# mako443/Text2Pos-CVPR2022

Hardware: AMD Instinct MI355X
Metric: cells+queries encoded/sec and top-k retrieval QPS, 256-pt cells, 12k-cell DB (higher is better)
Workload: dtype f16x3 (fp32 operands split hi+lo into fp16, 3 f16 MFMAs, fp32 accumulate; fp32-class error) for the encoders / f64 MFMA for the ranking

## Files before the change

### include/t2p.h

```cpp
#ifndef T2P_H
#define T2P_H
#include <stddef.h>
#include <stdint.h>

#ifdef __cplusplus
extern "C" {
#endif

#define T2P_ABI_VERSION 31
#define T2P_DEFAULT_CHUNK_OBJECTS 65000
#define T2P_MAX_CHUNK_OBJECTS 65535
#define T2P_TUNING_MASK 0x5
#define T2P_E_ARG (-1)
#define T2P_E_WORKSPACE (-2)
#define T2P_E_UNSUPPORTED (-3)

typedef void* t2p_stream_t;

int t2p_abi_version(void);
const char* t2p_last_error(void);

typedef struct t2p_cell_weights {
    const float* sa_w1[3];
    const float* sa_b1[3];
    const float* sa_w2[3];
    const float* sa_b2[3];
    const float* ga_w1;
    const float* ga_b1;
    const float* ga_w2;
    const float* ga_b2;
    const float* lin1_w;
    const float* lin1_b;
    const float* lin2_w;
    const float* lin2_b;
    const float* pn_w;
    const float* pn_b;
    const float* col_w1;
    const float* col_b1;
    const float* col_w2;
    const float* col_b2;
    const float* pos_w1;
    const float* pos_b1;
    const float* pos_w2;
    const float* pos_b2;
    const float* merge_w;
// ... 224 lines not shown
```

### profiles/tail_rows_census.py

```python
#!/usr/bin/env python
import argparse
import os
import sys

import numpy as np

sys.path.insert(0, os.path.join(os.path.dirname(os.path.abspath(__file__)), ".."))

RADII = (0.2, 0.3, 0.4)
MAX_NBR = 32


def level(pos: np.ndarray, r: float):
    n_d = pos.shape[0]
    n_c = (n_d + 1) // 2
    r2 = np.float32(r) * np.float32(r)
    mind = np.full(n_d, np.inf, dtype=np.float32)
    fps = np.zeros(n_c, dtype=np.int64)
    cnt = np.zeros(n_c, dtype=np.int64)
    cur = 0
    for c in range(n_c):
        fps[c] = cur
        d = pos - pos[cur]
        d2 = (d[:, 0] * d[:, 0] + d[:, 1] * d[:, 1]) + d[:, 2] * d[:, 2]
        cnt[c] = min(int((d2 < r2).sum()), MAX_NBR)
        mind = np.minimum(mind, d2)
        cur = int(np.argmax(mind))
    return fps, cnt


def dedup_hits(pos: np.ndarray, rgb: np.ndarray, fps: np.ndarray, r: float) -> int:
    key = np.concatenate([pos, rgb], axis=1).view(np.uint32)
    _, first = np.unique(key, axis=0, return_index=True)
    orig = np.zeros(pos.shape[0], dtype=bool)
    orig[first] = True
    r2 = np.float32(r) * np.float32(r)
    kept = 0
    for c in fps:
        d = pos - pos[c]
        d2 = (d[:, 0] * d[:, 0] + d[:, 1] * d[:, 1]) + d[:, 2] * d[:, 2]
        hits = np.flatnonzero(d2 < r2)[:MAX_NBR]
        kept += int(orig[hits].sum())
    return kept


def main():
    ap = argparse.ArgumentParser(description=__doc__.split("\n")[0])
    ap.add_argument("--seed", type=int, default=20220002, help="bench.py's object stream")
    ap.add_argument("--objects", type=int, default=3000)
    args = ap.parse_args()
    from importlib import import_module
    S = import_module("text2pos-cvpr2022_amd.synthetic")
    xyz, rgb, _, _ = S.make_objects(args.seed, 0, args.objects)
    n = xyz.shape[0]
    rows = np.zeros(3)
    rows_dedup = 0.0
    with_tail = np.zeros(3)
    tail_cent = np.zeros(3)
    tail_rows = np.zeros(3)
    executed = np.zeros(3)
    cents = np.zeros(3)
    for o in range(n):
        pos = xyz[o].astype(np.float32)
        for l in range(3):
            fps, cnt = level(pos, RADII[l])
            n_c = fps.shape[0]
            tail = (fps == 0) & (np.arange(n_c) > 0)
            all_rows = cnt.sum() + n_c
            t_rows = cnt[tail].sum()
            rows[l] += all_rows
            cents[l] += n_c
            with_tail[l] += tail.any()
            tail_cent[l] += tail.sum()
            tail_rows[l] += t_rows
            executed[l] += all_rows - t_rows + (cnt[0] if tail.any() else 0)
            if l == 0:
                rows_dedup += dedup_hits(pos, rgb[o].astype(np.float32), fps, RADII[0]) + n_c
            pos = pos[fps]
    print(f"{n} objects of seed {args.seed}")
    print("level | rows/object | objects with a tail | tail centroids | tail rows (non-self) | rows/object, tail shared")
    for l in range(3):
        extra = f" ({rows_dedup / n:.0f} after point dedup)" if l == 0 else ""
        print(f"SA{l + 1}   | {rows[l] / n:8.0f}{extra} | {100 * with_tail[l] / n:5.1f} % | {100 * tail_cent[l] / cents[l]:5.1f} % | "
              f"{100 * tail_rows[l] / rows[l]:5.1f} % | {executed[l] / n:8.0f} ({100 * (executed[l] / rows[l] - 1):+.1f} %)")


if __name__ == "__main__":
    main()
```

### text2pos-cvpr2022_amd/csrc/api.hip

```cpp
#include <stdarg.h>
#include <stdlib.h>
#include <string.h>

#include <mutex>
#include <set>
#include <utility>

#include "../../include/t2p.h"
#include "t2p_common.h"

namespace t2p {

static thread_local char g_err[512] = "";

void set_error(const char* fmt, ...) {
    va_list ap;
    va_start(ap, fmt);
    vsnprintf(g_err, sizeof(g_err), fmt, ap);
    va_end(ap);
}

int num_cus() {
    static int cached = 0;
    if (cached == 0) {
// ... 243 lines not shown
        GroupTables gt = ws.gt;
        const bool want_nbr = tr != nullptr && (tr->nbr[0] || tr->nbr[1] || tr->nbr[2] || tr->cnt[0] || tr->cnt[1] || tr->cnt[2]);
        if (!want_nbr)
            for (int l = 0; l < 3; l++) gt.nbr[l] = gt.cnt[l] = nullptr;
        for (int l = 0; l < 3; l++) {
            const int cf = l == 0 ? 3 : Geo::C[l - 1];
            gt.B[l] = lds_btab[l] ? nullptr : ws.B[l];
            gt.wp[l] = W.sa_w1[l] + (size_t)cf * Geo::H[l];
            gt.H[l] = Geo::H[l];
            gt.tail[l] = ws.F[l];
            gt.ld_tail[l] = Geo::LD[l];
            gt.tail_col0[l] = Geo::C[l];
        }
        gt.tail_rows[2] = g.gp;
        gt.A1 = sa1_points ? nullptr : ws.A[0];
        gt.w1 = W.sa_w1[0];
        gt.b1 = W.sa_b1[0];
        gt.rgb = rgb;
        gt.H1 = Geo::H[0];
        gt.guard = guard;

        SaParams bp[3] = {};
        for (int l = 0; l < 3; l++) {
            bp[l].n_rows = gt.n_rows[l];
            bp[l].n_obj = n;
            bp[l].prefix_ws = ws.prefix[l];
            bp[l].bounds_ws = ws.bounds[l];
            bp[l].W_x3 = cfg.precision == 1 ? W.sa_w2_x3[l] : nullptr;
            bp[l].wp = lds_btab[l] ? W.sa_w1[l] : nullptr;
            bp[l].n_dense = g.nd[l];
            bp[l].n_cent = g.nc[l];
        }
        bp[0].w1 = sa1_points ? W.sa_w1[0] : nullptr;
        for (int l = 0; l < 3; l++) gt.share_tail[l] = sa_shares_tail_rows(l, Geo::H[l], Geo::C[l], bp[l], cfg.n_pts, cfg.tuning) ? 1 : 0;

        T2P_TRY(launch_sample_group(xyz, n, cfg.n_pts, cfg.radius, gt, st));
        if (!(cfg.tuning & 1) && cfg.n_pts == 256)
            T2P_TRY(launch_dedup_rows(xyz, rgb, n, cfg.n_pts, gt.rows[0], gt.n_rows[0], g.nc[0], st));
        T2P_TRY(launch_sa_balance_levels(bp, Geo::H, Geo::C, st));
    }

    for (int l = 0; l < 3; l++) {
        const int H = Geo::H[l], C = Geo::C[l];
        const int cf = l == 0 ? 3 : Geo::C[l - 1];
        const float* pos_src = l == 0 ? xyz : ws.F[l - 1];
        const int ld_pos = l == 0 ? 3 : Geo::LD[l - 1];
        const int pos_col0 = l == 0 ? 0 : Geo::C[l - 1];
        if (l != 0) {
            WsParams p{};
            p.A = ws.F[l - 1];
            p.lda = Geo::LD[l - 1];
            p.k_live = Geo::C[l - 1] + 4;
            p.W = W.sa_w1[l];
            p.W_x3 = cfg.precision == 1 ? W.sa_w1_x3[l] : nullptr;
            p.ldw = H;
            p.bias = W.sa_b1[l];
            p.out = ws.A[l];
            p.ldo = H;
            p.relu = 0;
            p.M = n * g.nd[l];
            p.amax_out = gslot(l == 1 ? G_A2 : G_A3);
            T2P_TRY(launch_ws(WS_DENSE_STORE, Geo::LD[l - 1] - (cfg.precision == 1 ? 16 : 0), H, p, st));
        }
        SaParams p{};
        p.A = ws.A[l];
        p.Bc = ws.B[l];
        p.wp = lds_btab[l] ? W.sa_w1[l] + (size_t)cf * Geo::H[l] : nullptr;
// ... 651 lines not shown
    for (int l = 0; l < 3; l++) {
        gt.fps_idx[l] = fps_idx[l];
        gt.nbr[l] = nbr[l];
        gt.cnt[l] = cnt[l];
        gt.rows[l] = nullptr;
        gt.n_rows[l] = nullptr;
        gt.n_dense[l] = g.nd[l];
        gt.n_cent[l] = g.nc[l];
    }
    return launch_sample_group(xyz, n_obj, n_pts, radius_host, gt, (hipStream_t)stream);
}

int t2p_group_rows(const float* xyz, int64_t n_obj, int32_t n_pts, const float* radius_host, int32_t self_loops,
                   uint8_t* const* fps_idx, uint16_t* const* rows, uint16_t* const* n_rows, t2p_stream_t stream) {
    T2P_CHECK_ARG(xyz && radius_host && fps_idx && rows && n_rows, "group_rows: NULL argument");
    Geo g(n_pts);
    GroupTables gt{};
    gt.self_loops = self_loops ? 1 : 0;
    for (int l = 0; l < 3; l++) {
        T2P_CHECK_ARG(fps_idx[l] && rows[l] && n_rows[l], "group_rows: NULL table of level %d", l);
        gt.fps_idx[l] = fps_idx[l];
        gt.rows[l] = rows[l];
        gt.n_rows[l] = n_rows[l];
        gt.n_dense[l] = g.nd[l];
        gt.n_cent[l] = g.nc[l];
    }
    return launch_sample_group(xyz, n_obj, n_pts, radius_host, gt, (hipStream_t)stream);
}

int t2p_group_rows_shared(const float* xyz, int64_t n_obj, int32_t n_pts, const float* radius_host, int32_t self_loops,
                          int32_t share_mask, uint8_t* const* fps_idx, uint16_t* const* rows, uint16_t* const* n_rows,
                          t2p_stream_t stream) {
    T2P_CHECK_ARG(xyz && radius_host && fps_idx && rows && n_rows, "group_rows_shared: NULL argument");
    T2P_CHECK_ARG((share_mask & ~2) == 0, "group_rows_shared: share_mask=%#x (bit 1: SA level 2; no other level has a shared form)", share_mask);
    T2P_CHECK_ARG(share_mask == 0 || n_pts == 256, "group_rows_shared: shared lists exist for 256 points per object (n_pts = %d)", n_pts);
    Geo g(n_pts);
    GroupTables gt{};
    gt.self_loops = self_loops ? 1 : 0;
    for (int l = 0; l < 3; l++) {
        T2P_CHECK_ARG(fps_idx[l] && rows[l] && n_rows[l], "group_rows_shared: NULL table of level %d", l);
        gt.fps_idx[l] = fps_idx[l];
        gt.rows[l] = rows[l];
        gt.n_rows[l] = n_rows[l];
        gt.n_dense[l] = g.nd[l];
        gt.n_cent[l] = g.nc[l];
        gt.share_tail[l] = (share_mask >> l) & 1;
    }
    return launch_sample_group(xyz, n_obj, n_pts, radius_host, gt, (hipStream_t)stream);
}

int t2p_edge_counts(const uint16_t* rows, const uint16_t* n_rows, const int32_t* first_obj, int64_t n_obj, int32_t n_dense,
                    int32_t n_cent, int32_t self_loops, int32_t* counts, t2p_stream_t stream) {
    T2P_CHECK_ARG(n_obj >= 0 && (n_obj == 0 || (rows && n_rows && first_obj && counts)), "edge_counts: NULL argument");
    return launch_edge_counts(rows, n_rows, first_obj, n_obj, n_dense, n_cent, self_loops, counts, (hipStream_t)stream);
}

int t2p_edge_expand(const uint16_t* rows, const uint16_t* n_rows, const int32_t* first_obj, const int32_t* cent_ptr, int64_t n_obj,
                    int32_t n_dense, int32_t n_cent, int32_t self_loops, int32_t* src, int32_t* dst, t2p_stream_t stream) {
    T2P_CHECK_ARG(n_obj >= 0 && (n_obj == 0 || (rows && n_rows && first_obj && cent_ptr)), "edge_expand: NULL argument");
    return launch_edge_expand(rows, n_rows, first_obj, cent_ptr, n_obj, n_dense, n_cent, self_loops, src, dst, (hipStream_t)stream);
}

int t2p_pack_objects(const float* raw_xyz, const float* raw_rgb, const int32_t* obj_ptr, const int32_t* sample_idx,
                     const float* rot_cos_sin, int64_t n_obj, int32_t n_pts, float* xyz, float* rgb, float* center, float* mean_rgb,
                     t2p_stream_t stream) {
    T2P_CHECK_ARG(raw_xyz && raw_rgb && obj_ptr && sample_idx && xyz && rgb && center && mean_rgb, "pack_objects: NULL argument");
    T2P_CHECK_ARG(n_obj >= 0 && n_pts >= 1, "pack_objects: bad sizes");
// ... 53 lines not shown
```

### text2pos-cvpr2022_amd/csrc/sa_points.hip

```cpp
#ifndef T2P_PABL
#define T2P_PABL 0
#endif
#include "t2p_common.h"

namespace t2p {
namespace {

typedef uint32_t u32x4 __attribute__((ext_vector_type(4)));
typedef uint32_t u32x2 __attribute__((ext_vector_type(2)));
typedef float f32x2 __attribute__((ext_vector_type(2)));

#define MFMA16(a, b, c) __builtin_amdgcn_mfma_f32_32x32x16_f16(a, b, c, 0, 0, 0)
#define MFMA8(a, b, c) __builtin_amdgcn_mfma_f32_32x32x8f16(a, b, c, 0, 0, 0)

template <int NW>
struct PtsCfg {
    static constexpr int K = 32, N = 64, NC = 128, ND = 256, GS = 16;
    static constexpr int NT = 64 * NW;
    static constexpr int S16 = K / 16, NTW = N / 32;
    static constexpr int HS = GS / 2, NH = NC / HS;
    static constexpr int MAXR = NC * 33;
    static constexpr int LPR = 64 / HS;
    static constexpr int ACC_BYTES = GS * N * 4;
    static constexpr int PTS_BYTES = ND * 24;
    static constexpr int SELF_BYTES = GS * 24;
    static constexpr int CEN_BYTES = GS * 32;
    static constexpr int RING_BYTES = 4 * 64 * 2;
    static constexpr int WAVE_BYTES = ACC_BYTES + PTS_BYTES + SELF_BYTES + CEN_BYTES + 16 + 64 + RING_BYTES;
    static_assert(WAVE_BYTES % 16 == 0, "16-byte accesses");
    static constexpr size_t lds_bytes() { return (size_t)NW * WAVE_BYTES + 16 + N * 4; }
};

__device__ __forceinline__ float relu1(float v) {
    const int b = __float_as_int(v);
    return __int_as_float(b > 0 ? b : 0);
}
__device__ __forceinline__ void split2(float v0, float v1, uint32_t& hi, uint32_t& lo) {
    const fp16x2 hh = cvt_pk_f16(v0, v1);
    const fp16x2 ll = cvt_pk_f16(sub_half<0>(v0, hh), sub_half<1>(v1, hh));
    hi = __builtin_bit_cast(uint32_t, hh);
    lo = __builtin_bit_cast(uint32_t, ll);
}

template <int NW, int PARTS>
__global__ __launch_bounds__(64 * NW, (NW + 3) / 4) void k_sa_points(SaParams p) {
    using C = PtsCfg<NW>;
    static_assert(PARTS == 1 || (C::NH % PARTS == 0 && C::NH / PARTS >= 3), "a part is a whole number (>= 3: two open + one fetched ahead) of halves");
    constexpr int K = C::K, N = C::N, NC = C::NC;
    extern __shared__ __attribute__((aligned(16))) char lds[];
    const int tid = threadIdx.x, lane = tid & 63;
    const int wave = __builtin_amdgcn_readfirstlane(tid >> 6);
    const int h = lane >> 5, rr = lane & 31;
    const uint32_t acc_off = (uint32_t)(wave * C::WAVE_BYTES);
    const uint32_t pts_off = acc_off + C::ACC_BYTES;
    const uint32_t self_off = pts_off + C::PTS_BYTES;
    const uint32_t cen_off = self_off + C::SELF_BYTES;
    const uint32_t one_off = cen_off + C::CEN_BYTES;
    const uint32_t dst_off = one_off + 16;
    const uint32_t ring_off = dst_off + 64;
    if (lane == 0) *(f32x4*)(lds + one_off) = f32x4{1.f, 0.f, 0.f, 0.f};

    half8 w_hi[C::NTW][C::S16], w_lo[C::NTW][C::S16];
    {
        const uint4* wp = (const uint4*)p.W_x3;
        constexpr int PLANE_U4 = (N / 32) * C::S16 * 64;
#pragma unroll
        for (int nt = 0; nt < C::NTW; nt++)
#pragma unroll
            for (int s = 0; s < C::S16; s++) {
                uint4 pc[2][2];
#pragma unroll
                for (int hp = 0; hp < 2; hp++) {
                    const int kb = 16 * s + 8 * hp;
                    const int half_ = kb / (K / 2), step_ = (kb % (K / 2)) / 8;
                    const int idx = (((nt * C::S16 + step_) * 2 + half_) * 32) + rr;
                    pc[0][hp] = wp[idx];
                    pc[1][hp] = wp[PLANE_U4 + idx];
                }
                const u32x4 vh = h ? u32x4{pc[0][0].z, pc[0][0].w, pc[0][1].z, pc[0][1].w} : u32x4{pc[0][0].x, pc[0][0].y, pc[0][1].x, pc[0][1].y};
                const u32x4 vl = h ? u32x4{pc[1][0].z, pc[1][0].w, pc[1][1].z, pc[1][1].w} : u32x4{pc[1][0].x, pc[1][0].y, pc[1][1].x, pc[1][1].y};
                w_hi[nt][s] = __builtin_bit_cast(half8, vh);
                w_lo[nt][s] = __builtin_bit_cast(half8, vl);
            }
    }
    half4 w1_hi, w1_lo;
    {
        float wv[4];
#pragma unroll
        for (int e = 0; e < 4; e++) {
            const int k = 4 * h + e;
            wv[e] = k < 6 ? p.w1[k * K + rr] : (k == 6 ? p.b1[rr] : 0.f);
        }
// ... 26 lines not shown
        const int g = g_begin + (PARTS > 1 ? gi / PARTS : gi);
        if (g >= g_end) break;
        constexpr int HP = C::NH / PARTS;
        const int hs = PARTS > 1 ? (gi % PARTS) * HP : 0;
        const int hend = hs + HP;
        int n = __builtin_amdgcn_readfirstlane((int)p.n_rows[g]);
        const uint16_t* list = p.rows + (int64_t)g * C::MAXR;
        if constexpr (PARTS > 1) {
            auto lower = [&](int target) -> int {
                if (target <= 0 || n <= 0) return 0;
                if (target >= NC) return n;
                const int step = (n + 63) >> 6;
                const int i0 = lane * step;
                const uint32_t c0 = i0 < n ? (((uint32_t)list[i0] >> 8) & 127u) : 255u;
                const unsigned long long ge = __ballot(c0 >= (uint32_t)target);
                const int fl = ge ? (int)__builtin_ctzll(ge) : 64;
                if (fl == 0) return 0;
                int hi = fl * step;
                hi = hi < n ? hi : n;
                const int base = (fl - 1) * step + 1;
                for (int b = base; b < hi; b += 64) {
                    const int i = b + lane;
                    const uint32_t c = i < hi ? (((uint32_t)list[i] >> 8) & 127u) : 255u;
                    const unsigned long long m = __ballot(c >= (uint32_t)target);
                    if (m) return b + (int)__builtin_ctzll(m);
                }
                return hi;
            };
            const int r_lo = __builtin_amdgcn_readfirstlane(lower(hs * C::HS));
            const int r_hi = __builtin_amdgcn_readfirstlane(lower(hend * C::HS));
            list += r_lo;
            n = r_hi - r_lo;
        }
        const int first = __builtin_amdgcn_readfirstlane(p.first[g]);
        const uint32_t sb0 = (uint32_t)(first * C::ND + (g - first) * NC);

        const int nwin = (n + 63) >> 6;
        auto load_win = [&](int w) -> uint32_t {
            int i = w * 64 + lane;
            i = i < n ? i : n - 1;
            i = i > 0 ? i : 0;
            return (uint32_t)list[i];
        };
        auto ring_write = [&](int w, uint32_t v) { *(uint16_t*)(lds + ring_off + (((w & 3) * 64 + lane) * 2)) = (uint16_t)v; };
        auto ring_read = [&](int r) -> uint32_t {
            return (uint32_t) * (const uint16_t*)(lds + ring_off + (((r + rr) & 255) * 2));
        };
        const uint32_t win0 = load_win(0), win1 = load_win(1);
        uint32_t pend = load_win(2);
        int w_loaded = 2;

        typedef float f32x3 __attribute__((ext_vector_type(3)));
        struct Side { f32x3 q, sp, sc; };
        auto fetch_side = [&](int hh) -> Side {
            const int c = hh * C::HS + (lane & (C::HS - 1));
            const float* pc = p.out + ((int64_t)g * NC + c) * (int64_t)p.ldo + N;
            const int64_t ai = (int64_t)sb0 + c;
            return Side{*(const f32x3*)pc, *(const f32x3*)(p.pos_src + ai * 3), *(const f32x3*)(p.feat_src + ai * 3)};
        };
        const Side side0 = fetch_side(hs), side1 = fetch_side(hs + 1);

        {
            const f32x4* px4 = (const f32x4*)(p.pos_src + (int64_t)g * C::ND * 3) + lane * 3;
            const f32x4* pc4 = (const f32x4*)(p.feat_src + (int64_t)g * C::ND * 3) + lane * 3;
            const f32x4 a0 = px4[0], a1 = px4[1], a2 = px4[2];
            const f32x4 c0_ = pc4[0], c1_ = pc4[1], c2_ = pc4[2];
            f32x4* rec = (f32x4*)(lds + pts_off + lane * 96);
            rec[0] = f32x4{c0_[0], c0_[1], c0_[2], a0[0]};
            rec[1] = f32x4{a0[1], a0[2], c0_[3], c1_[0]};
            rec[2] = f32x4{c1_[1], a0[3], a1[0], a1[1]};
            rec[3] = f32x4{c1_[2], c1_[3], c2_[0], a1[2]};
            rec[4] = f32x4{a1[3], a2[0], c2_[1], c2_[2]};
            rec[5] = f32x4{c2_[3], a2[1], a2[2], a2[3]};
        }
        ring_write(0, win0);
        ring_write(1, win1);

        auto flush_out = [&]() {
            if (has_pout) {
#pragma unroll
                for (int q4 = 0; q4 < NPL / 4; q4++) *(f32x4*)(pptr + q4 * 4) = pout[q4];
                has_pout = false;
            }
        };
        auto drain = [&](int hh, bool live) {
            flush_out();
            pptr = p.out + ((int64_t)g * NC + hh * C::HS + cr) * (int64_t)p.ldo + cs * NPL;
            const uint32_t a0 = acc_off + (uint32_t)((((hh & 1) * C::HS + cr) * N + cs * NPL) * 4);
            int top = gtop;
#pragma unroll
            for (int q4 = 0; q4 < NPL / 4; q4++) {
                f32x4 v = f32x4{0.f, 0.f, 0.f, 0.f};
                if (live) {
                    const f32x4 raw = *(const f32x4*)(lds + a0 + q4 * 16);
                    const f32x4 bq = *(const f32x4*)(lds + bias_off + q4 * 16);
#pragma unroll
                    for (int e = 0; e < 4; e++) {
                        const float r = fmaxf(raw[e] + bq[e], 0.f);
                        const int bits = __float_as_int(r);
                        top = bits > top ? bits : top;
                        v[e] = r * p.out_scale;
                    }
                }
                pout[q4] = v;
            }
            has_pout = true;
            gtop = top;
        };
        auto open_half = [&](int hh, const Side& sd) {
            const uint32_t s0 = (uint32_t)((hh & 1) * C::HS);
            if (lane < C::HS) {
                uint2* sp = (uint2*)(lds + self_off + (s0 + lane) * 24);
                sp[0] = uint2{__float_as_uint(sd.sc[0]), __float_as_uint(sd.sc[1])};
                sp[1] = uint2{__float_as_uint(sd.sc[2]), __float_as_uint(sd.sp[0])};
                sp[2] = uint2{__float_as_uint(sd.sp[1]), __float_as_uint(sd.sp[2])};
                f32x4* cp = (f32x4*)(lds + cen_off + (s0 + lane) * 32);
                cp[0] = f32x4{0.f, 0.f, 0.f, sd.q[0]};
                cp[1] = f32x4{sd.q[1], sd.q[2], 0.f, 0.f};
            }
            typedef int i32x4 __attribute__((ext_vector_type(4)));
            const uint32_t a0 = acc_off + (uint32_t)(((s0 + cr) * N + cs * NPL) * 4);
#pragma unroll
            for (int q4 = 0; q4 < NPL / 4; q4++)
                *(i32x4*)(lds + a0 + q4 * 16) = i32x4{(int)0xFF800000, (int)0xFF800000, (int)0xFF800000, (int)0xFF800000};
        };

        open_half(hs, side0);
        open_half(hs + 1, side1);
        Side side_n = fetch_side(hs + 2);
        int hf = hs + 2;
        int hd = hs, ho = hs + 2;
        int r0 = 0;
        uint32_t e_cur = n > 0 ? ring_read(0) : 0u;
        while (r0 < n) {
            const uint32_t key = r0 + rr < n ? ((e_cur >> 8) & 127u) : 255u;
            const int h0 = __builtin_amdgcn_readfirstlane((int)key) >> 3;
            const uint32_t over = (uint32_t)__ballot(key >= (uint32_t)((h0 + 2) * C::HS));
            const int c = over ? (int)__builtin_ctz(over) : 32;
            const uint32_t e_nxt = ring_read(r0 + c);
            if (hd < h0 || ho < h0 + 2) {
                if (hd < h0) asm volatile("s_waitcnt lgkmcnt(0)" ::: "memory");
                while (hd < h0) {
                    drain(hd, hd < ho);
                    hd++;
                }
                if (ho < hd) ho = hd;
                const int want = h0 + 2 < hend ? h0 + 2 : hend;
                while (ho < want) {
                    if (hf != ho) side_n = fetch_side(ho);
                    open_half(ho, side_n);
                    ho++;
                    if (ho < hend) {
                        side_n = fetch_side(ho);
                        hf = ho;
                    }
                }
            }
            if (w_loaded * 64 < r0 + 96 && w_loaded < nwin) {
                ring_write(w_loaded, pend);
                w_loaded++;
                flush_out();
                if (w_loaded < nwin) pend = load_win(w_loaded);
            }
            const uint32_t m = rr < c ? e_cur : (uint32_t)__builtin_amdgcn_readlane((int)e_cur, c - 1);
            const uint32_t src = m & 0xFFu, d = m >> 8;
            const uint32_t dl = d & 15u;
            const uint32_t rec = (d & 0x80u) ? self_off + dl * 24u : pts_off + src * 24u;
            const uint32_t pa0 = rec + (uint32_t)(h * 16), pa1 = h ? one_off : rec + 8u;
            f32x4 pv, cv;
            if constexpr (T2P_PABL & 8) {
                pv = f32x4{(float)pa0, 1.f, 2.f, (float)pa1};
                cv = f32x4{(float)dl, 1.f, 2.f, 3.f};
            } else {
                const f32x2 p0 = *(const f32x2*)(lds + pa0), p1 = *(const f32x2*)(lds + pa1);
                pv = f32x4{p0[0], p0[1], p1[0], p1[1]};
                cv = *(const f32x4*)(lds + cen_off + dl * 32u + (uint32_t)(h * 16));
            }
            *(uint16_t*)(lds + dst_off + rr * 2) = (uint16_t)(dl * (uint32_t)(N * 4));
            uint32_t xh[2], xl[2];
            split2(pv[0] - cv[0], pv[1] - cv[1], xh[0], xl[0]);
            split2(pv[2] - cv[2], pv[3] - cv[3], xh[1], xl[1]);
            const half4 x_hi = __builtin_bit_cast(half4, u32x2{xh[0], xh[1]});
            const half4 x_lo = __builtin_bit_cast(half4, u32x2{xl[0], xl[1]});
            f32x16 hid;
            if constexpr (T2P_PABL & 4) {
#pragma unroll
                for (int e = 0; e < 16; e++) hid[e] = (float)x_hi[e & 3] + (float)x_lo[e & 3];
            } else {
// ... 36 lines not shown
                    const uint32_t pair = (e & 2) ? four[e >> 2].y : four[e >> 2].x;
                    ad[e] = acc_off + (uint32_t)(rr * 4) + ((e & 1) ? (pair >> 16) : (pair & 0xFFFFu));
                }
                static_assert(C::NTW == 2, "the hazard fence below names both result blocks");
                asm volatile("s_nop 15" : "+v"(acc[0]), "+v"(acc[1])::"memory");
#pragma unroll
                for (int nt = 0; nt < C::NTW; nt++)
#pragma unroll
                    for (int e = 0; e < 16; e++)
                        if constexpr (!(T2P_PABL & 1))
                            asm volatile("ds_max_f32 %0, %1 offset:%2" ::"v"(ad[e]), "v"(acc[nt][e]), "n"(nt * 128) : "memory");
                        else
                            asm volatile("; %0 %1" ::"v"(ad[e]), "v"(acc[nt][e]));
            }
            r0 += c;
            e_cur = e_nxt;
        }
        asm volatile("s_waitcnt lgkmcnt(0)" ::: "memory");
        for (; hd < hend; hd++) drain(hd, hd < ho);
        flush_out();
    }
    uint32_t gbits = 0;
    guard_track_bits(gbits, gtop);
    if (p.amax_out != nullptr && lane == 0 && gbits != 0u)
        atomicMax(p.amax_out, __float_as_uint(__uint_as_float(gbits) * p.out_scale));
}

#ifndef T2P_PTS_WAVES
#define T2P_PTS_WAVES 12
#endif
constexpr int kPtsWaves = T2P_PTS_WAVES;
constexpr int kPtsParts = 4;

}

bool sa_points_selected(int H, int Cout, const SaParams& p) {
    return H == 32 && Cout == 64 && p.W_x3 != nullptr && p.wp != nullptr && p.w1 != nullptr;
}

int sa_points_launch_shape(int64_t n_obj, int* tile_rows, int* n_wg) {
    int n = num_cus();
    if (n > 1024) n = 1024;
    if (n > n_obj) n = (int)n_obj;
    *tile_rows = 32;
    *n_wg = n;
    return 0;
}

int launch_sa_points(int H, int Cout, const SaParams& p, hipStream_t st) {
    if (!(H == 32 && Cout == 64 && p.n_cent == 128 && p.n_dense == 256 && p.wp && p.W_x3 && p.w1 && p.b1 && p.feat_src && p.pos_src &&
          p.ld_pos == 3 && p.pos_col0 == 0)) {
        set_error("sa_points: built for SA level 1 (6 -> 32 -> 64, 128 centroids of 256 points [xyz] + [rgb], f16x3)");
        return T2P_E_UNSUPPORTED;
    }
    using C = PtsCfg<kPtsWaves>;
    auto kern = k_sa_points<kPtsWaves, 1>, kern_parts = k_sa_points<kPtsWaves, kPtsParts>;
    T2P_TRY(reserve_lds((const void*)kern, C::lds_bytes(), "sa_points"));
    T2P_TRY(reserve_lds((const void*)kern_parts, C::lds_bytes(), "sa_points"));
    if (p.n_obj <= 0) return 0;
    T2P_CHECK_ARG(p.n_obj < (1 << 22), "sa_points: chunk too large");
    T2P_CHECK_ARG((((uintptr_t)p.pos_src | (uintptr_t)p.feat_src | (uintptr_t)p.out | (uintptr_t)p.W_x3) & 15) == 0 && p.ldo % 4 == 0,
                  "sa_points: points, output rows and weights must be 16-byte aligned");
    int tr, n_wg;
    sa_points_launch_shape(p.n_obj, &tr, &n_wg);
    if (!p.balanced) T2P_TRY(launch_sa_balance(p, tr, n_wg, st));
    ProfScope ps_("ws_edge_sa_k32_n64", st);
    const bool parts = p.n_obj * 2 <= (int64_t)n_wg * kPtsWaves;
    T2P_REPEAT(ps_) hipLaunchKernelGGL(parts ? kern_parts : kern, dim3(n_wg), dim3(C::NT), C::lds_bytes(), st, p);
    T2P_CHECK_LAUNCH("sa_points");
    return 0;
}

}
```

### text2pos-cvpr2022_amd/csrc/sample_group.hip

```cpp
#include "t2p_common.h"

namespace t2p {

#pragma clang fp contract(off)

namespace {

#ifndef T2P_FPS_PK
#define T2P_FPS_PK 1
#endif

constexpr int kMaxPts = 256;
constexpr int kMaxNbr = 32;

__device__ __forceinline__ float dist2(float ax, float ay, float az, float bx, float by, float bz) {
#pragma clang fp contract(off)
    float dx = ax - bx, dy = ay - by, dz = az - bz;
    float xx = dx * dx, yy = dy * dy, zz = dz * dz;
    float s = xx + yy;
    return s + zz;
}

template <int CTRL>
__device__ __forceinline__ int dpp_i(int v) {
// ... 78 lines not shown
            lower = __builtin_amdgcn_mbcnt_hi((uint32_t)(m >> 32), __builtin_amdgcn_mbcnt_lo((uint32_t)m, lower));
            count += __popcll(m);
        }
        int pos = lower;
#pragma unroll
        for (int j = 0; j < PPL; j++) {
            if (hit[j] && pos < kMaxNbr) {
                const int i = lane * PPL + j;
                if (nbr_lds) nbr_lds[c * kMaxNbr + pos] = (uint8_t)i;
                if (rows_out) rows_out[base + pos] = (uint16_t)((c << 8) | i);
            }
            pos += hit[j] ? 1 : 0;
        }
        const int kept = count < kMaxNbr ? count : kMaxNbr;
        if (lane == 0) {
            if (nbr_lds) cnt_lds[c] = (uint8_t)kept;
            if (self_loops && rows_out) rows_out[base + kept] = (uint16_t)(((c | 0x80) << 8) | c);
        }
        base += kept + (self_loops ? 1 : 0);
        if (c + 1 < n_c) {
            const float mx = wave_max_f(bd);
            const unsigned long long tie = __ballot(bd == mx);
            cur = __builtin_amdgcn_readlane(bi, (int)__builtin_ctzll(tie));
        }
    }
    if (rows_out && lane < 4 && base + lane < n_c * (kMaxNbr + 1)) rows_out[base + lane] = 0xFFFF;
    *n_rows_out = base;
    __syncthreads();
}

template <int PPL, bool SHARE = false>
__device__ void level_fast(const float* px, const float* py, const float* pz, int n_c, float r2, uint8_t* sel, float* qx,
                           float* qy, float* qz, uint16_t* __restrict__ rows_out, int self_loops, int* n_rows_out,
                           int tail_code = 0) {
    const int lane = threadIdx.x;
    const int i0 = lane * PPL;
    float x[PPL], y[PPL], z[PPL];
    uint32_t mind[PPL];
#pragma unroll
    for (int j = 0; j < PPL; j++) {
        x[j] = px[i0 + j];
        y[j] = py[i0 + j];
        z[j] = pz[i0 + j];
        mind[j] = 0x7f800000u;
    }
    int cur = 0;
    int base = 0;
    [[maybe_unused]] bool tail_open = false;
    for (int c = 0; c < n_c; c++) {
        const float cx = px[cur], cy = py[cur], cz = pz[cur];
        if (lane == 0) {
            sel[c] = (uint8_t)cur;
            qx[c] = cx;
            qy[c] = cy;
            qz[c] = cz;
        }
        bool tail = false;
        if constexpr (SHARE) {
            tail = c > 0 && cur == 0;
            if (tail && tail_open) {
                if (self_loops && lane == 0) rows_out[(uint32_t)base] = (uint16_t)(((c | 0x80) << 8) | c);
                base += self_loops ? 1 : 0;
                continue;
            }
            tail_open = tail;
        }
        float d[PPL];
        unsigned long long m[PPL];
        if constexpr (T2P_FPS_PK && PPL % 2 == 0) {
            typedef float f32x2 __attribute__((ext_vector_type(2)));
            const f32x2 c2x = {cx, cx}, c2y = {cy, cy}, c2z = {cz, cz};
#pragma unroll
            for (int j = 0; j < PPL; j += 2) {
#pragma clang fp contract(off)
                const f32x2 dx = f32x2{x[j], x[j + 1]} - c2x, dy = f32x2{y[j], y[j + 1]} - c2y, dz = f32x2{z[j], z[j + 1]} - c2z;
                const f32x2 xx = dx * dx, yy = dy * dy, zz = dz * dz;
                const f32x2 sxy = xx + yy;
                const f32x2 dd = sxy + zz;
                d[j] = dd[0];
                d[j + 1] = dd[1];
            }
// ... 6 lines not shown
#pragma unroll
            for (int j = 0; j < PPL; j++) {
                d[j] = dist2(x[j], y[j], z[j], cx, cy, cz);
                mind[j] = min(mind[j], __float_as_uint(d[j]));
                m[j] = __ballot(d[j] < r2);
            }
        }
        int lower = 0, count = 0;
#pragma unroll
        for (int j = 0; j < PPL; j++) {
            lower = __builtin_amdgcn_mbcnt_hi((uint32_t)(m[j] >> 32), __builtin_amdgcn_mbcnt_lo((uint32_t)m[j], lower));
            count += __popcll(m[j]);
        }
        const uint32_t tag = (uint32_t)(tail ? tail_code : c) << 8;
        char* const rows_b = (char*)rows_out;
        if (count <= kMaxNbr) {
            uint32_t off = 2u * (uint32_t)(base + lower);
#pragma unroll
            for (int j = 0; j < PPL; j++) {
                const bool hit = d[j] < r2;
                if (hit) *(uint16_t*)(rows_b + off) = (uint16_t)(tag | (uint32_t)(i0 + j));
                off += hit ? 2u : 0u;
            }
        } else {
            uint32_t pos = (uint32_t)lower;
#pragma unroll
            for (int j = 0; j < PPL; j++) {
                const bool hit = d[j] < r2;
                if (hit && pos < (uint32_t)kMaxNbr) *(uint16_t*)(rows_b + 2u * ((uint32_t)base + pos)) = (uint16_t)(tag | (uint32_t)(i0 + j));
                pos += hit ? 1u : 0u;
            }
        }
        const int kept = count < kMaxNbr ? count : kMaxNbr;
        if (self_loops && lane == 0) rows_out[(uint32_t)(base + kept)] = (uint16_t)(((c | 0x80) << 8) | c);
        base += kept + (self_loops ? 1 : 0);
        if (c + 1 < n_c) {
            uint32_t bd = mind[0];
#pragma unroll
            for (int j = 1; j < PPL; j++) bd = max(bd, mind[j]);
            const uint32_t mx = wave_max_u(bd);
            const unsigned long long tie = __ballot(bd == mx);
            int jb = PPL - 1;
#pragma unroll
            for (int j = PPL - 2; j >= 0; j--) jb = mind[j] == mx ? j : jb;
            cur = __builtin_amdgcn_readlane(i0 + jb, (int)__builtin_ctzll(tie));
        }
    }
    if (lane < 4 && base + lane < n_c * (kMaxNbr + 1)) rows_out[base + lane] = 0xFFFF;
    *n_rows_out = base;
    __syncthreads();
}

__device__ __attribute__((noinline)) void emit_centroid_table(const float* qx, const float* qy, const float* qz, int n_c,
                                                    const float* __restrict__ wp, int H, float* __restrict__ out,
                                                    float* __restrict__ tail, int ld_tail, int tail_col0, int tail_quads,
                                                    int tail_rows) {
    const int lane = threadIdx.x;
    if (tail != nullptr) {
        const int hq = lane % tail_quads;
        for (int c = n_c + lane / tail_quads; c < tail_rows; c += 64 / tail_quads)
            *(f32x4*)(tail + (size_t)c * ld_tail + tail_col0 + hq * 4) =
                hq == 0 ? f32x4{qx[n_c - 1], qy[n_c - 1], qz[n_c - 1], 0.f} : f32x4{0.f, 0.f, 0.f, 0.f};
    }
    if (out == nullptr) {
        if (tail == nullptr) return;
        const int hq = lane % tail_quads;
        for (int c = lane / tail_quads; c < n_c; c += 64 / tail_quads)
            *(f32x4*)(tail + (size_t)c * ld_tail + tail_col0 + hq * 4) =
                hq == 0 ? f32x4{qx[c], qy[c], qz[c], 0.f} : f32x4{0.f, 0.f, 0.f, 0.f};
        return;
    }
    const int tpr = H >> 2, rpp = 64 / tpr, hq = lane % tpr;
    const f32x4 w0 = *(const f32x4*)(wp + hq * 4), w1 = *(const f32x4*)(wp + H + hq * 4), w2 = *(const f32x4*)(wp + 2 * H + hq * 4);
    for (int c = lane / tpr; c < n_c; c += rpp) {
        const float px = qx[c], py = qy[c], pz = qz[c];
        f32x4 v;
#pragma unroll
        for (int e = 0; e < 4; e++) {
// ... 57 lines not shown
            if (gt.rgb != nullptr) {
                const float* col = gt.rgb + o * (int64_t)n_pts * 3;
                for (int i = lane; i < n_pts * 3; i += 64) {
                    const uint32_t b = __float_as_uint(col[i]) & 0x7fffffffu;
                    in_bits = b > in_bits ? b : in_bits;
                }
            }
            guard_publish_bits_above(gt.guard + G_INPUT, in_bits, 0x3f800000u);
        }
        __syncthreads();
        if (gt.A1 != nullptr) {
            const float *w1 = gt.w1, *b1 = gt.b1;
            asm volatile("" : "+s"(w1), "+s"(b1));
            emit_point_table(p0, p0 + kMaxPts, p0 + 2 * kMaxPts, gt.rgb + o * (int64_t)n_pts * 3, n_pts, w1, b1, gt.H1,
                             gt.A1 + o * (int64_t)n_pts * gt.H1);
        }
        float* pin[4][3] = {{p0, p0 + kMaxPts, p0 + 2 * kMaxPts},
                            {p1, p1 + kMaxPts / 2, p1 + kMaxPts},
                            {p2, p2 + kMaxPts / 4, p2 + kMaxPts / 2},
                            {p3, p3 + kMaxPts / 8, p3 + kMaxPts / 4}};
        const float rr[3] = {r0 * r0, r1 * r1, r2 * r2};
#pragma unroll
        for (int l = 0; l < 3; l++) {
            const int n_d = gt.n_dense[l], n_c = gt.n_cent[l];
            if (want_nbr) {
                for (int i = lane; i < n_c * kMaxNbr / 4; i += 64) ((uint32_t*)nbr_lds)[i] = 0u;
            }
            __syncthreads();
            int n_rows = 0;
            uint16_t* g_rows16 = gt.rows[l] ? gt.rows[l] + o * (int64_t)(n_c * (kMaxNbr + 1)) : nullptr;
            if constexpr (FAST) {
                if (l == 0)
                    level_fast<4>(pin[l][0], pin[l][1], pin[l][2], n_c, rr[l], sel_lds, pin[l + 1][0], pin[l + 1][1],
                                  pin[l + 1][2], g_rows16, gt.self_loops, &n_rows);
                else if (l == 1 && gt.share_tail[1])
                    level_fast<2, true>(pin[l][0], pin[l][1], pin[l][2], n_c, rr[l], sel_lds, pin[l + 1][0], pin[l + 1][1],
                                        pin[l + 1][2], g_rows16, gt.self_loops, &n_rows, kSaTailCode);
                else if (l == 1)
                    level_fast<2>(pin[l][0], pin[l][1], pin[l][2], n_c, rr[l], sel_lds, pin[l + 1][0], pin[l + 1][1],
                                  pin[l + 1][2], g_rows16, gt.self_loops, &n_rows);
                else
                    level_fast<1>(pin[l][0], pin[l][1], pin[l][2], n_c, rr[l], sel_lds, pin[l + 1][0], pin[l + 1][1],
                                  pin[l + 1][2], g_rows16, gt.self_loops, &n_rows);
            } else if (n_d > 128)
                level<4>(pin[l][0], pin[l][1], pin[l][2], n_d, n_c, rr[l], sel_lds, pin[l + 1][0], pin[l + 1][1],
                         pin[l + 1][2], nbr_lds, cnt_lds, g_rows16, gt.self_loops, &n_rows);
            else if (n_d > 64)
                level<2>(pin[l][0], pin[l][1], pin[l][2], n_d, n_c, rr[l], sel_lds, pin[l + 1][0], pin[l + 1][1],
                         pin[l + 1][2], nbr_lds, cnt_lds, g_rows16, gt.self_loops, &n_rows);
            else
                level<1>(pin[l][0], pin[l][1], pin[l][2], n_d, n_c, rr[l], sel_lds, pin[l + 1][0], pin[l + 1][1],
                         pin[l + 1][2], nbr_lds, cnt_lds, g_rows16, gt.self_loops, &n_rows);
            if (g_rows16 != nullptr && lane == 0) gt.n_rows[l][o] = (uint16_t)n_rows;
            if (gt.B[l] != nullptr || gt.tail[l] != nullptr) {
                const float* wpl = gt.wp[l];
                asm volatile("" : "+s"(wpl));
                const int t_rows = gt.tail_rows[l] > n_c ? gt.tail_rows[l] : n_c;
                emit_centroid_table(pin[l + 1][0], pin[l + 1][1], pin[l + 1][2], n_c, wpl, gt.H[l],
                                    gt.B[l] ? gt.B[l] + o * (int64_t)n_c * gt.H[l] : nullptr,
                                    gt.tail[l] ? gt.tail[l] + o * (int64_t)t_rows * gt.ld_tail[l] : nullptr, gt.ld_tail[l],
                                    gt.tail_col0[l], l == 2 ? 8 : 1, t_rows);
            }
            uint8_t* g_sel = gt.fps_idx[l] + o * (int64_t)n_c;
            for (int i = lane; i < n_c; i += 64) g_sel[i] = sel_lds[i];
            if (want_nbr) {
                uint8_t* g_nbr = gt.nbr[l] + o * (int64_t)n_c * kMaxNbr;
                uint8_t* g_cnt = gt.cnt[l] + o * (int64_t)n_c;
// ... 134 lines not shown
```

### text2pos-cvpr2022_amd/csrc/t2p_common.h

```cpp
#pragma once
#include <hip/hip_runtime.h>
#include <stdint.h>
#include <stdio.h>

namespace t2p {

void set_error(const char* fmt, ...);

#define T2P_E_ARG (-1)
#define T2P_E_WORKSPACE (-2)
#define T2P_E_UNSUPPORTED (-3)

#define T2P_CHECK_ARG(cond, ...)                  \
    do {                                          \
        if (!(cond)) {                            \
            ::t2p::set_error(__VA_ARGS__);        \
            return T2P_E_ARG;                     \
        }                                         \
    } while (0)

#define T2P_CHECK_LAUNCH(name)                                                   \
    do {                                                                         \
        hipError_t e__ = hipGetLastError();                                      \
        if (e__ != hipSuccess) {                                                 \
// ... 209 lines not shown
};
int launch_ws(int mode, int K, int N, const WsParams& p, hipStream_t st);

struct SaParams {
    const float* A;
    const float* Bc;
    const float* wp;
    const float* W;
    const void* W_x3;
    const float* bias;
    float out_scale;
    float* out;
    int ldo;
    const uint16_t* rows;
    const uint16_t* n_rows;
    const int32_t* first;
    const uint8_t* fps_idx;
    const float* pos_src;
    int ld_pos, pos_col0;
    const float* feat_src;
    const float* w1;
    const float* b1;
    int n_dense, n_cent;
    int64_t n_obj;
    int32_t* prefix_ws;
    int32_t* bounds_ws;
    int balanced;
    uint32_t* amax_out;
    int out_rows;
};
int launch_ws_sa(int H, int C, const SaParams& p, hipStream_t st);
int launch_sa_balance(const SaParams& p, int tile_rows, int n_wg, hipStream_t st);
constexpr int kSaTailCode = 64;
bool sa_rows_selected(int H, int C, const SaParams& p);
int launch_sa_rows(int H, int C, const SaParams& p, hipStream_t st);
int sa_rows_launch_shape(int64_t n_obj, int* tile_rows, int* n_wg);
bool sa_points_selected(int H, int C, const SaParams& p);
int launch_sa_points(int H, int C, const SaParams& p, hipStream_t st);
int sa_points_launch_shape(int64_t n_obj, int* tile_rows, int* n_wg);
bool sa3_selected(int H, int C, const SaParams& p);
int launch_sa3(const SaParams& p, hipStream_t st);
int sa3_launch_shape(int64_t n_obj, int* tile_rows, int* n_wg);
inline bool sa_shares_tail_rows(int l, int H, int C, const SaParams& p, int n_pts, int tuning) {
    return l == 1 && n_pts == 256 && !(tuning & 4) && p.n_dense == 128 && p.n_cent == 64 && sa_rows_selected(H, C, p);
}
int launch_sa_balance_levels(const SaParams p[3], const int H[3], const int C[3], hipStream_t st);

int launch_bilstm_impl(const float* gate_table , const float* whh ,
                       const void* whh_x3 ,
                       float whh_scale, const int32_t* tokens , const int32_t* lengths, int B, int T, int V, int D,
                       float* hdir_ws , float* out ,
                       hipStream_t st);

int launch_lstm_cell_fwd(const float* pre, const float* table, const int32_t* tokens, const int32_t* lengths, int64_t B, int T,
                         int D, int step, int reverse, const float* c_prev, const float* h_prev, float* gates, float* c,
                         float* h, hipStream_t st);
int launch_lstm_cell_bwd(const float* dh_gemm, const float* dh_carry_in, const float* dc_in, const float* gates,
                         const float* c_prev, const float* c, const int32_t* lengths, int64_t B, int D, int step, float* d_pre,
                         float* dc_out, float* dh_carry_out, hipStream_t st);

size_t bn_train_workspace_bytes(int64_t rows, int n_seg, int C);
int launch_bn_relu_train_forward(const float* x, const int32_t* seg_ptr, int n_seg, int64_t rows, int C, const float* gamma,
                                 const float* beta, float eps, int relu, float* y, float* mean, float* invstd,
                                 float* var_unbiased, double* part, hipStream_t st);
int launch_bn_relu_train_backward(const float* dy, const float* x, const float* beta, const int32_t* seg_ptr, int n_seg,
                                  int64_t rows, int C, const float* mean, const float* invstd, const float* gamma, int relu,
                                  float* dx, float* dgamma_seg, float* dbeta_seg, double* part, hipStream_t st);
int launch_edge_feat_fwd(const float* x, const float* pos, const float* pos_c, const int32_t* src, const int32_t* dst, int64_t E,
                         int C, int W, float* out, hipStream_t st);
int launch_edge_feat_bwd(const float* dout, const int32_t* src, int64_t E, int C, int W, float* dx, hipStream_t st);
int launch_pair_feat_fwd(const float* x, const int32_t* tgt, const int32_t* src, int64_t E, int D, float* out, hipStream_t st);
int launch_pair_feat_bwd(const float* dout, const int32_t* tgt, const int32_t* src, int64_t E, int D, float* dx, hipStream_t st);
int launch_segment_mean(const float* x, const int32_t* seg_ptr, int n_seg, int C, float* out, hipStream_t st);
int launch_segment_mean_backward(const float* dout, const int32_t* seg_ptr, int n_seg, int C, float* dx, hipStream_t st);
int launch_rownorm_bwd(const float* x, const float* dy, int64_t n_rows, int dim, float* dx, hipStream_t st);
int launch_segment_max(const float* x, const int32_t* seg_ptr, int n_seg, int C, float* out, int32_t* arg, hipStream_t st);
// ... 15 lines not shown
```

Before: 152,800.

## Share SA1 tail-centroid neighbor rows via snapshot instead of recomputing duplicates

Extends tail-row sharing to SA level 1. Once farthest-point sampling returns to point 0, the grouping step stops emitting neighbor lists for the remaining centroids, whose lists would all be identical, and writes them as self-loop-only rows. The first tail centroid gets a marked self-loop row. The points SA kernel snapshots that centroid's max-pooled accumulator into LDS and merges it into the later tail centroids. This cuts the number of MLP rows executed in SA1. In exchange it adds LDS space per wave, extra branches and a waitcnt in the hot loop, and it applies only when whole objects are processed per wave, self-loops are on and the tuning bit is clear.

Result: no change. 153,100 (median of 6 runs) (+0.2%).

```diff
diff --git a/include/t2p.h b/include/t2p.h
--- a/include/t2p.h
+++ b/include/t2p.h
@@ -10,7 +10,7 @@
 #define T2P_ABI_VERSION 31
 #define T2P_DEFAULT_CHUNK_OBJECTS 65000
 #define T2P_MAX_CHUNK_OBJECTS 65535
-#define T2P_TUNING_MASK 0x5
+#define T2P_TUNING_MASK 0xD
 #define T2P_E_ARG (-1)
 #define T2P_E_WORKSPACE (-2)
 #define T2P_E_UNSUPPORTED (-3)
diff --git a/profiles/sa1_rows_executed.py b/profiles/sa1_rows_executed.py
--- /dev/null
+++ b/profiles/sa1_rows_executed.py
@@ -0,0 +1,40 @@
+#!/usr/bin/env python
+import argparse
+import os
+import sys
+
+import numpy as np
+import torch
+
+sys.path.insert(0, os.path.join(os.path.dirname(os.path.abspath(__file__)), ".."))
+
+
+def main():
+    ap = argparse.ArgumentParser(description=__doc__.split("\n")[0])
+    ap.add_argument("--seed", type=int, default=20220002, help="bench.py's object stream")
+    ap.add_argument("--cells", type=int, default=12000)
+    args = ap.parse_args()
+    from importlib import import_module
+    S = import_module("text2pos-cvpr2022_amd.synthetic")
+    ops = import_module("text2pos-cvpr2022_amd.ops")
+    xyz, rgb, _, _, cell_ptr = S.make_cells(args.seed, args.cells)
+    dev = torch.device("cuda:0")
+    n = xyz.shape[0]
+    raw = 0
+    total = {0: 0, 1: 0}
+    for a in range(0, n, 8192):
+        x = torch.from_numpy(xyz[a:a + 8192]).to(dev)
+        c = torch.from_numpy(rgb[a:a + 8192]).to(dev)
+        for mask in (0, 1):
+            g = ops.group_rows(x, self_loops=True, share_mask=mask)
+            if mask == 0:
+                raw += int(g["n_rows"][0].cpu().numpy().view(np.uint16).astype(np.int64).sum())
+            ops.dedup_rows(x, c, g["rows"][0], g["n_rows"][0])
+            total[mask] += int(g["n_rows"][0].cpu().numpy().view(np.uint16).astype(np.int64).sum())
+    print(f"{n} objects / {len(cell_ptr) - 1} cells")
+    print(f"SA1 rows per step: raw {raw} ({raw / n:.1f} per object), after point dedup {total[0]} ({total[0] / n:.1f}), "
+          f"tail shared {total[1]} ({total[1] / n:.1f}): {100 * (total[1] / total[0] - 1):+.2f} %")
+
+
+if __name__ == "__main__":
+    main()
diff --git a/profiles/tail_rows_census.py b/profiles/tail_rows_census.py
--- a/profiles/tail_rows_census.py
+++ b/profiles/tail_rows_census.py
@@ -29,18 +29,18 @@
     return fps, cnt
 
 
-def dedup_hits(pos: np.ndarray, rgb: np.ndarray, fps: np.ndarray, r: float) -> int:
+def dedup_hits(pos: np.ndarray, rgb: np.ndarray, fps: np.ndarray, r: float) -> np.ndarray:
     key = np.concatenate([pos, rgb], axis=1).view(np.uint32)
     _, first = np.unique(key, axis=0, return_index=True)
     orig = np.zeros(pos.shape[0], dtype=bool)
     orig[first] = True
     r2 = np.float32(r) * np.float32(r)
-    kept = 0
-    for c in fps:
+    kept = np.zeros(len(fps), dtype=np.int64)
+    for i, c in enumerate(fps):
         d = pos - pos[c]
         d2 = (d[:, 0] * d[:, 0] + d[:, 1] * d[:, 1]) + d[:, 2] * d[:, 2]
         hits = np.flatnonzero(d2 < r2)[:MAX_NBR]
-        kept += int(orig[hits].sum())
+        kept[i] = int(orig[hits].sum())
     return kept
 
 
@@ -55,6 +55,7 @@
     n = xyz.shape[0]
     rows = np.zeros(3)
     rows_dedup = 0.0
+    exec_dedup = 0.0
     with_tail = np.zeros(3)
     tail_cent = np.zeros(3)
     tail_rows = np.zeros(3)
@@ -75,7 +76,12 @@
             tail_rows[l] += t_rows
             executed[l] += all_rows - t_rows + (cnt[0] if tail.any() else 0)
             if l == 0:
-                rows_dedup += dedup_hits(pos, rgb[o].astype(np.float32), fps, RADII[0]) + n_c
+                kept = dedup_hits(pos, rgb[o].astype(np.float32), fps, RADII[0])
+                rows_dedup += kept.sum() + n_c
+                later = tail.copy()
+                if tail.any():
+                    later[np.argmax(tail)] = False
+                exec_dedup += kept.sum() + n_c - kept[later].sum()
             pos = pos[fps]
     print(f"{n} objects of seed {args.seed}")
     print("level | rows/object | objects with a tail | tail centroids | tail rows (non-self) | rows/object, tail shared")
@@ -83,6 +89,8 @@
         extra = f" ({rows_dedup / n:.0f} after point dedup)" if l == 0 else ""
         print(f"SA{l + 1}   | {rows[l] / n:8.0f}{extra} | {100 * with_tail[l] / n:5.1f} % | {100 * tail_cent[l] / cents[l]:5.1f} % | "
               f"{100 * tail_rows[l] / rows[l]:5.1f} % | {executed[l] / n:8.0f} ({100 * (executed[l] / rows[l] - 1):+.1f} %)")
+    print(f"SA1 after point dedup: {rows_dedup / n:.0f} rows/object with full lists, {exec_dedup / n:.0f} with the tail shared "
+          f"({100 * (exec_dedup / rows_dedup - 1):+.1f} %)")
 
 
 if __name__ == "__main__":
diff --git a/text2pos-cvpr2022_amd/csrc/api.hip b/text2pos-cvpr2022_amd/csrc/api.hip
--- a/text2pos-cvpr2022_amd/csrc/api.hip
+++ b/text2pos-cvpr2022_amd/csrc/api.hip
@@ -299,7 +299,8 @@
             bp[l].n_cent = g.nc[l];
         }
         bp[0].w1 = sa1_points ? W.sa_w1[0] : nullptr;
-        for (int l = 0; l < 3; l++) gt.share_tail[l] = sa_shares_tail_rows(l, Geo::H[l], Geo::C[l], bp[l], cfg.n_pts, cfg.tuning) ? 1 : 0;
+        for (int l = 0; l < 3; l++)
+            gt.share_tail[l] = sa_shares_tail_rows(l, Geo::H[l], Geo::C[l], bp[l], cfg.n_pts, cfg.tuning, cfg.self_loops) ? 1 : 0;
 
         T2P_TRY(launch_sample_group(xyz, n, cfg.n_pts, cfg.radius, gt, st));
         if (!(cfg.tuning & 1) && cfg.n_pts == 256)
@@ -1017,7 +1018,8 @@
                           int32_t share_mask, uint8_t* const* fps_idx, uint16_t* const* rows, uint16_t* const* n_rows,
                           t2p_stream_t stream) {
     T2P_CHECK_ARG(xyz && radius_host && fps_idx && rows && n_rows, "group_rows_shared: NULL argument");
-    T2P_CHECK_ARG((share_mask & ~2) == 0, "group_rows_shared: share_mask=%#x (bit 1: SA level 2; no other level has a shared form)", share_mask);
+    T2P_CHECK_ARG((share_mask & ~3) == 0, "group_rows_shared: share_mask=%#x (bit 0: SA level 1, bit 1: SA level 2; level 3 has no shared form)", share_mask);
+    T2P_CHECK_ARG(!(share_mask & 1) || self_loops, "group_rows_shared: level 1's shared form marks a self-loop row: self_loops must be set");
     T2P_CHECK_ARG(share_mask == 0 || n_pts == 256, "group_rows_shared: shared lists exist for 256 points per object (n_pts = %d)", n_pts);
     Geo g(n_pts);
     GroupTables gt{};
diff --git a/text2pos-cvpr2022_amd/csrc/sa_points.hip b/text2pos-cvpr2022_amd/csrc/sa_points.hip
--- a/text2pos-cvpr2022_amd/csrc/sa_points.hip
+++ b/text2pos-cvpr2022_amd/csrc/sa_points.hip
@@ -26,7 +26,8 @@
     static constexpr int SELF_BYTES = GS * 24;
     static constexpr int CEN_BYTES = GS * 32;
     static constexpr int RING_BYTES = 4 * 64 * 2;
-    static constexpr int WAVE_BYTES = ACC_BYTES + PTS_BYTES + SELF_BYTES + CEN_BYTES + 16 + 64 + RING_BYTES;
+    static constexpr int SNAP_BYTES = N * 4;
+    static constexpr int WAVE_BYTES = ACC_BYTES + PTS_BYTES + SELF_BYTES + CEN_BYTES + 16 + 64 + RING_BYTES + SNAP_BYTES;
     static_assert(WAVE_BYTES % 16 == 0, "16-byte accesses");
     static constexpr size_t lds_bytes() { return (size_t)NW * WAVE_BYTES + 16 + N * 4; }
 };
@@ -58,6 +59,7 @@
     const uint32_t one_off = cen_off + C::CEN_BYTES;
     const uint32_t dst_off = one_off + 16;
     const uint32_t ring_off = dst_off + 64;
+    [[maybe_unused]] const uint32_t snap_off = ring_off + C::RING_BYTES;
     if (lane == 0) *(f32x4*)(lds + one_off) = f32x4{1.f, 0.f, 0.f, 0.f};
 
     half8 w_hi[C::NTW][C::S16], w_lo[C::NTW][C::S16];
@@ -150,6 +152,7 @@
             list += r_lo;
             n = r_hi - r_lo;
         }
+        [[maybe_unused]] int t_first = NC;
         const int first = __builtin_amdgcn_readfirstlane(p.first[g]);
         const uint32_t sb0 = (uint32_t)(first * C::ND + (g - first) * NC);
 
@@ -210,7 +213,16 @@
             for (int q4 = 0; q4 < NPL / 4; q4++) {
                 f32x4 v = f32x4{0.f, 0.f, 0.f, 0.f};
                 if (live) {
-                    const f32x4 raw = *(const f32x4*)(lds + a0 + q4 * 16);
+                    f32x4 raw = *(const f32x4*)(lds + a0 + q4 * 16);
+                    if constexpr (PARTS == 1) {
+                        if (hh * C::HS + C::HS - 1 > t_first) {
+                            const f32x4 sq = *(const f32x4*)(lds + snap_off + (uint32_t)((cs * NPL + q4 * 4) * 4));
+                            if (hh * C::HS + cr > t_first) {
+#pragma unroll
+                                for (int e = 0; e < 4; e++) raw[e] = fmaxf(raw[e], sq[e]);
+                            }
+                        }
+                    }
                     const f32x4 bq = *(const f32x4*)(lds + bias_off + q4 * 16);
 #pragma unroll
                     for (int e = 0; e < 4; e++) {
@@ -253,7 +265,14 @@
         while (r0 < n) {
             const uint32_t key = r0 + rr < n ? ((e_cur >> 8) & 127u) : 255u;
             const int h0 = __builtin_amdgcn_readfirstlane((int)key) >> 3;
-            const uint32_t over = (uint32_t)__ballot(key >= (uint32_t)((h0 + 2) * C::HS));
+            bool beyond = key >= (uint32_t)((h0 + 2) * C::HS);
+            [[maybe_unused]] bool snap_now = false;
+            if constexpr (PARTS == 1) {
+                const bool marked = (e_cur & 0x80FFu) == (0x8000u | (uint32_t)kSaTailMark) && key != 255u;
+                beyond = beyond || (marked && rr != 0);
+                snap_now = ((uint32_t)__builtin_amdgcn_readfirstlane((int)e_cur) & 0x80FFu) == (0x8000u | (uint32_t)kSaTailMark);
+            }
+            const uint32_t over = (uint32_t)__ballot(beyond);
             const int c = over ? (int)__builtin_ctz(over) : 32;
             const uint32_t e_nxt = ring_read(r0 + c);
             if (hd < h0 || ho < h0 + 2) {
@@ -272,6 +291,14 @@
                         side_n = fetch_side(ho);
                         hf = ho;
                     }
+                }
+            }
+            if constexpr (PARTS == 1) {
+                if (snap_now) {
+                    asm volatile("s_waitcnt lgkmcnt(0)" ::: "memory");
+                    t_first = __builtin_amdgcn_readfirstlane((int)key);
+                    const float v = *(const float*)(lds + acc_off + (uint32_t)((((t_first & (C::GS - 1)) * N) + lane) * 4));
+                    *(float*)(lds + snap_off + (uint32_t)(lane * 4)) = v;
                 }
             }
             if (w_loaded * 64 < r0 + 96 && w_loaded < nwin) {
@@ -374,6 +401,12 @@
 constexpr int kPtsWaves = T2P_PTS_WAVES;
 constexpr int kPtsParts = 4;
 
+}
+
+bool sa_points_whole_objects(int64_t n_obj) {
+    int tr, n_wg;
+    sa_points_launch_shape(n_obj, &tr, &n_wg);
+    return !(n_obj * 2 <= (int64_t)n_wg * kPtsWaves);
 }
 
 bool sa_points_selected(int H, int Cout, const SaParams& p) {
@@ -407,7 +440,7 @@
     sa_points_launch_shape(p.n_obj, &tr, &n_wg);
     if (!p.balanced) T2P_TRY(launch_sa_balance(p, tr, n_wg, st));
     ProfScope ps_("ws_edge_sa_k32_n64", st);
-    const bool parts = p.n_obj * 2 <= (int64_t)n_wg * kPtsWaves;
+    const bool parts = !sa_points_whole_objects(p.n_obj);
     T2P_REPEAT(ps_) hipLaunchKernelGGL(parts ? kern_parts : kern, dim3(n_wg), dim3(C::NT), C::lds_bytes(), st, p);
     T2P_CHECK_LAUNCH("sa_points");
     return 0;
diff --git a/text2pos-cvpr2022_amd/csrc/sample_group.hip b/text2pos-cvpr2022_amd/csrc/sample_group.hip
--- a/text2pos-cvpr2022_amd/csrc/sample_group.hip
+++ b/text2pos-cvpr2022_amd/csrc/sample_group.hip
@@ -134,7 +134,7 @@
 template <int PPL, bool SHARE = false>
 __device__ void level_fast(const float* px, const float* py, const float* pz, int n_c, float r2, uint8_t* sel, float* qx,
                            float* qy, float* qz, uint16_t* __restrict__ rows_out, int self_loops, int* n_rows_out,
-                           int tail_code = 0) {
+                           int tail_code = 0, int mark = 0) {
     const int lane = threadIdx.x;
     const int i0 = lane * PPL;
     float x[PPL], y[PPL], z[PPL];
@@ -149,6 +149,9 @@
     int cur = 0;
     int base = 0;
     [[maybe_unused]] bool tail_open = false;
+    [[maybe_unused]] const int mark_pt = mark ? 0 : -1;
+    [[maybe_unused]] bool first_tail = false;
+    [[maybe_unused]] int c_tail = n_c;
     for (int c = 0; c < n_c; c++) {
         const float cx = px[cur], cy = py[cur], cz = pz[cur];
         if (lane == 0) {
@@ -221,8 +224,15 @@
             }
         }
         const int kept = count < kMaxNbr ? count : kMaxNbr;
-        if (self_loops && lane == 0) rows_out[(uint32_t)(base + kept)] = (uint16_t)(((c | 0x80) << 8) | c);
+        if (self_loops && lane == 0)
+            rows_out[(uint32_t)(base + kept)] = (uint16_t)(((c | 0x80) << 8) | (first_tail ? 0xFF : c));
         base += kept + (self_loops ? 1 : 0);
+        if constexpr (!SHARE && PPL == 4) {
+            if (first_tail) {
+                c_tail = c + 1;
+                break;
+            }
+        }
         if (c + 1 < n_c) {
             uint32_t bd = mind[0];
 #pragma unroll
@@ -233,6 +243,20 @@
 #pragma unroll
             for (int j = PPL - 2; j >= 0; j--) jb = mind[j] == mx ? j : jb;
             cur = __builtin_amdgcn_readlane(i0 + jb, (int)__builtin_ctzll(tie));
+            if constexpr (!SHARE && PPL == 4) first_tail = cur == mark_pt;
+        }
+    }
+    if constexpr (!SHARE && PPL == 4) {
+        if (c_tail < n_c) {
+            const float cx = px[0], cy = py[0], cz = pz[0];
+            for (int c = c_tail + lane; c < n_c; c += 64) {
+                sel[c] = 0;
+                qx[c] = cx;
+                qy[c] = cy;
+                qz[c] = cz;
+                rows_out[(uint32_t)(base + (c - c_tail))] = (uint16_t)(((c | 0x80) << 8) | c);
+            }
+            base += n_c - c_tail;
         }
     }
     if (lane < 4 && base + lane < n_c * (kMaxNbr + 1)) rows_out[base + lane] = 0xFFFF;
@@ -356,7 +380,7 @@
             if constexpr (FAST) {
                 if (l == 0)
                     level_fast<4>(pin[l][0], pin[l][1], pin[l][2], n_c, rr[l], sel_lds, pin[l + 1][0], pin[l + 1][1],
-                                  pin[l + 1][2], g_rows16, gt.self_loops, &n_rows);
+                                  pin[l + 1][2], g_rows16, gt.self_loops, &n_rows, 0, gt.share_tail[0] && gt.self_loops);
                 else if (l == 1 && gt.share_tail[1])
                     level_fast<2, true>(pin[l][0], pin[l][1], pin[l][2], n_c, rr[l], sel_lds, pin[l + 1][0], pin[l + 1][1],
                                         pin[l + 1][2], g_rows16, gt.self_loops, &n_rows, kSaTailCode);
diff --git a/text2pos-cvpr2022_amd/csrc/t2p_common.h b/text2pos-cvpr2022_amd/csrc/t2p_common.h
--- a/text2pos-cvpr2022_amd/csrc/t2p_common.h
+++ b/text2pos-cvpr2022_amd/csrc/t2p_common.h
@@ -265,16 +265,21 @@
 int launch_ws_sa(int H, int C, const SaParams& p, hipStream_t st);
 int launch_sa_balance(const SaParams& p, int tile_rows, int n_wg, hipStream_t st);
 constexpr int kSaTailCode = 64;
+constexpr int kSaTailMark = 0xFF;
 bool sa_rows_selected(int H, int C, const SaParams& p);
 int launch_sa_rows(int H, int C, const SaParams& p, hipStream_t st);
 int sa_rows_launch_shape(int64_t n_obj, int* tile_rows, int* n_wg);
 bool sa_points_selected(int H, int C, const SaParams& p);
 int launch_sa_points(int H, int C, const SaParams& p, hipStream_t st);
 int sa_points_launch_shape(int64_t n_obj, int* tile_rows, int* n_wg);
+bool sa_points_whole_objects(int64_t n_obj);
 bool sa3_selected(int H, int C, const SaParams& p);
 int launch_sa3(const SaParams& p, hipStream_t st);
 int sa3_launch_shape(int64_t n_obj, int* tile_rows, int* n_wg);
-inline bool sa_shares_tail_rows(int l, int H, int C, const SaParams& p, int n_pts, int tuning) {
+inline bool sa_shares_tail_rows(int l, int H, int C, const SaParams& p, int n_pts, int tuning, int self_loops) {
+    if (l == 0)
+        return n_pts == 256 && !(tuning & 8) && self_loops && p.n_dense == 256 && p.n_cent == 128 && sa_points_selected(H, C, p) &&
+               sa_points_whole_objects(p.n_obj);
     return l == 1 && n_pts == 256 && !(tuning & 4) && p.n_dense == 128 && p.n_cent == 64 && sa_rows_selected(H, C, p);
 }
 int launch_sa_balance_levels(const SaParams p[3], const int H[3], const int C[3], hipStream_t st);
```
